# drnatebrown/col-bwt

Measured on AMD Instinct MI355X. Metric: query bases/s, higher is better.
Workload: dtype int64

## Files before the change

### col-bwt_amd/csrc/fat2_query.hip

```cpp
#include <hip/hip_runtime.h>
#include <stdint.h>
#include <stdlib.h>
#include <string.h>

#include <algorithm>

#include "device_layout.h"
#include "fat_cursor.h"
#include "fat_layout.h"
#include "lane_io.h"
#include "lane_out.h"
#include "query_kernels.h"

namespace colbwt {

namespace {

constexpr uint32_t kOffMis0 = 0xFFFFFFFCu;
constexpr uint32_t kOffMis1 = 0xFFFFFFFBu;

#ifdef COLBWT_COUNT_TRIPS
#define FAT2_STAT(k) (++stat[k])
#else
#define FAT2_STAT(k) ((void)0)
#endif

__device__ __forceinline__ uint32_t mis_slot(const uint8_t *top, uint32_t own, uint32_t c) {
    const uint32_t aidx = top[own], cidx = top[c];
    const uint32_t slot = cidx < aidx ? cidx : cidx - 1;
    return cidx < 4 && slot < kFatSlots ? slot : kFatSlots;
}

template <int K, typename PmlT, bool kDeep>
__global__ __launch_bounds__(kQueryBlock)
void fat2_query_kernel(FatTable T, const uint8_t *__restrict__ bases, const uint64_t *__restrict__ read_off,
                       uint64_t n_reads, uint32_t big_reads, uint32_t tail_permille,
                       PmlT *__restrict__ pml, uint8_t *__restrict__ cid) {
    constexpr bool kWide = sizeof(PmlT) == 4;
    __shared__ uint4 s_stage[kWaves][8][64];
    __shared__ uint4 s_win[kWaves][4][64];
    __shared__ uint32_t s_claim;
    __shared__ uint8_t s_top[256];
    const uint32_t wave = threadIdx.x >> 6, lane = threadIdx.x & 63u, g8 = lane & ~7u, p = lane & 7u;
    uint32_t *const s_jx = reinterpret_cast<uint32_t *>(&s_stage[wave][7][48]);
    ChunkPlan plan;
    plan.init(n_reads, big_reads, tail_permille);
    if (threadIdx.x == 0) s_claim = 0;
    s_top[threadIdx.x] = (uint8_t)fat_top_index(T.top4, threadIdx.x);
    __syncthreads();
    uint32_t *const claim = &s_claim;
    ReadCursor rc;
    bool done;
    rc.c_next = threadIdx.x;
    rc.request_chunk(plan, read_off);
    rc.commit();
    done = !rc.enter_chunk(plan, claim);

    OutRuns acc;
    uint32_t trip = 0;
    LaneWindow win;
    win.init(rc.off + rc.k - 1);
    uint4 (*const my_win)[64] = s_win[wave];

    uint32_t j = done ? 0u : T.r - 1;
    uint32_t o = kOffLastPos;
    uint32_t L = 0;
    const uint4 *const my_row = &s_stage[wave][p][g8];

#ifdef COLBWT_COUNT_TRIPS
    unsigned long long stat[8] = {0, 0, 0, 0, 0, 0, 0, 0};
#endif
    while (__any(!done)) {
        bool step_back = false;
        if (!done && rc.k == 0 && !rc.next_in_flight && (rc.r != rc.r_lo || rc.nc_ready)) {
            if (rc.r != rc.r_lo) {
                rc.r -= 1;
                rc.k = rc.off - rc.next_off;
                rc.off = rc.next_off;
                step_back = rc.r > rc.r_lo;
            } else if (kWide || acc.cnt == 0) {
                done = !rc.enter_chunk(plan, claim);
                if (!done) win.init(rc.off + rc.k - 1);
            }
            j = done ? 0u : T.r - 1;
            o = kOffLastPos;
            L = 0;
        }
        const bool live = !done && rc.k != 0;
        uint64_t &k = rc.k;
        const uint64_t g = rc.off + k - 1;

        s_jx[lane] = j;
        wave_sync();
        {
            const uint4 ja = *reinterpret_cast<const uint4 *>(&s_jx[g8]);
            const uint4 jb = *reinterpret_cast<const uint4 *>(&s_jx[g8 + 4]);
            const uint32_t jq[8] = {ja.x, ja.y, ja.z, ja.w, jb.x, jb.y, jb.z, jb.w};
            wave_sync();
#pragma unroll
            for (uint32_t q = 0; q < 8; ++q)
                __builtin_amdgcn_global_load_lds(T.lines + (uint64_t)jq[q] * kFatRowBytes + ((p ^ q) << 4), &s_stage[wave][q][0],
                                                 16, 0, 0);
        }
        if (live && win.avail(g) < (k < 8u ? (uint32_t)k : 8u)) win.request(my_win, bases, g);
        if (step_back) { rc.in_next = read_off[rc.r - 1]; rc.next_in_flight = true; }
        if (!done && rc.fetch_pending) rc.request_chunk(plan, read_off);
        lds_dma_landed();
        rc.commit();

        const uint32_t have = live ? win.avail(g) : 0u;
        uint32_t consumed = 0, l_new = 0, keep = 0xFFFFFFFFu, keep1 = 0xFFFFFFFFu;
        uint64_t ids = 0;
        if (!live || have == 0) FAT2_STAT(5);
        if (live && have != 0) {
            const uint64_t W = win.get8(my_win, lane, g);
            const uint32_t left = k < have ? (uint32_t)k : have;
            if (o == kOffMis0 || o == kOffMis1) {
                FAT2_STAT(2);
                const uint32_t h4 = !kDeep && o == kOffMis1 ? 4u : 0u;
                const uint4 e0 = my_row[(h4 + 0u) ^ p], e1 = my_row[(h4 + 1u) ^ p], e2 = my_row[(h4 + 2u) ^ p],
                            e3 = my_row[(h4 + 3u) ^ p];
                const uint32_t carry = L;
                const uint32_t t1 = (e0.y >> 16) & 0xFFu, d1 = e0.y >> 24, v1 = e3.z & 7u;
                uint32_t oc = 4;
                if (left >= 2) {
                    const uint32_t c2 = (uint32_t)(W >> 48) & 0xFFu;
                    const uint32_t s2 = mis_slot(s_top, t1, c2);
                    if (c2 == t1) oc = 0;
                    else if (s2 < kFatSlots && ((v1 >> s2) & 1u)) oc = 1 + s2;
                }
                if (oc < 4) {
                    const uint32_t J = oc == 0 ? e0.z : oc == 1 ? e0.w : oc == 2 ? e1.x : e1.y;
                    const uint32_t rho = oc == 0 ? e1.z : oc == 1 ? e1.w : oc == 2 ? e2.x : e2.y;
                    const uint32_t pw = oc < 2 ? e2.z : e2.w, P = (oc & 1u) ? pw >> 16 : pw & 0xFFFFu;
                    const uint32_t ch = (e3.x >> (8 * oc)) & 0xFFu, cd = (e3.y >> (8 * oc)) & 0xFFu;
                    const uint32_t vo = (e3.z >> (4 + 4 * oc)) & 7u;
                    consumed = 2;
                    l_new = 1;
                    keep = oc == 0 ? 0xFFFFFFFFu : 0u;
                    ids = (uint64_t)(d1 | (carry << 8));
                    L = oc == 0 ? 1u : 0u;
                    uint32_t nJ = J, nP = P, nrho = rho, nch = ch, ncd = cd, nv = vo, seen = 2;
                    if constexpr (kDeep) {
                        if (left >= 3 && ((uint32_t)(W >> 40) & 0xFFu) == ch) {
                            const uint4 f0 = my_row[4u ^ p], f1 = my_row[5u ^ p], f2 = my_row[6u ^ p], f3 = my_row[7u ^ p];
                            nJ = oc == 0 ? f0.x : oc == 1 ? f0.y : oc == 2 ? f0.z : f0.w;
                            nrho = oc == 0 ? f1.x : oc == 1 ? f1.y : oc == 2 ? f1.z : f1.w;
                            const uint32_t pw2 = oc < 2 ? f2.x : f2.y;
                            nP = (oc & 1u) ? pw2 >> 16 : pw2 & 0xFFFFu;
                            nch = (f2.z >> (8 * oc)) & 0xFFu;
                            ncd = (f2.w >> (8 * oc)) & 0xFFu;
                            nv = (f3.x >> (4 * oc)) & 7u;
                            consumed = 3;
                            seen = 3;
                            ids = (uint64_t)(cd | (d1 << 8) | (carry << 16));
                            if (oc == 0) { l_new = 2; keep = 0xFFFFFFFFu; }
                            else { l_new = 1; keep = 0xFFFFFFFFu; keep1 = 0u; }
                            L += 1;
                        }
                    }
                    if (k > consumed) {
                        uint32_t sn = kFatSlots;
                        if (left > seen) {
                            const uint32_t cn = (uint32_t)(W >> (8u * (7u - seen))) & 0xFFu;
                            if (cn != nch) sn = mis_slot(s_top, nch, cn);
                        }
                        if (sn < kFatSlots && ((nv >> sn) & 1u)) {
                            const uint32_t e = nrho * kFatSlots + sn;
                            j = T.slot_line0 + (kDeep ? e : e >> 1);
                            o = kDeep ? kOffMis0 : kOffMis0 - (e & 1u);
                            L = ncd;
                        } else {
                            j = nJ;
                            o = nP;
                        }
                    }
                } else {
                    consumed = 1;
                    l_new = 0;
                    ids = (uint64_t)carry;
                    L = 0;
                    j = e0.x;
                    o = e0.y & 0xFFFFu;
                }
            } else {
                FAT2_STAT(0);
                const uint4 r0 = my_row[0 ^ p];
                const uint4 r1 = my_row[1 ^ p];
                const uint64_t CH = (uint64_t)r0.x | ((uint64_t)r0.y << 32);
                const uint64_t CID = (uint64_t)r0.z | ((uint64_t)r0.w << 32);
                const uint32_t len = r1.x & 0xFFFFu;
                uint32_t skip = 0;
                bool stay = false;
                if (o == kOffPred) { o = len - 1; skip = 1; }
                else if (o == kOffSucc) { o = 0; skip = 1; }
                else if (o >= len && j < T.r - 1) {
                    o -= len;
                    j += 1;
                    stay = true;
                    FAT2_STAT(1);
                } else {
                    o = o < len ? o : len - 1;
                }
                if (!stay) {
                    const uint64_t X = skip ? ((W >> 8) ^ CH) & 0x00FFFFFFFFFFFFFFull : W ^ CH;
                    const uint32_t run = matching_top_bytes(X);
                    const uint32_t cap = left + skip < (uint32_t)K ? left + skip : (uint32_t)K;
                    uint32_t steps = run < cap ? run : cap;
                    bool own_jump = true, to_entry = false;
                    uint32_t e_next = 0, carry = 0;
                    if (run < cap) {
                        const uint32_t d = run + 1u, sh = 8u * (8u - d);
                        const uint32_t c = (uint32_t)(W >> (sh + 8u * skip)) & 0xFFu;
                        const uint32_t s = mis_slot(s_top, (uint32_t)(CH >> sh) & 0xFFu, c);
                        if (s < kFatSlots && ((r1.w >> (3u * run + s)) & 1u)) {
                            const uint32_t rho = reinterpret_cast<const uint32_t *>(&my_row[((kFatRho / 16) + (run >> 2)) ^ p])[run & 3u];
                            e_next = rho * kFatSlots + s;
                            carry = (uint32_t)(CID >> sh) & 0xFFu;
                            to_entry = true;
                            own_jump = false;
                        }
                    }
                    if (run == 0 && !to_entry) {
                        const uint32_t c = (uint32_t)(W >> 56);
                        const uint32_t cidx = T.cmap[c];
                        bool moved = false;
                        if (cidx != kAbsent) moved = fat_threshold_scan(T, j, o, c, cidx);
                        FAT2_STAT(moved ? 3 : 4);
                        if (moved) {
                            steps = 1;
                            consumed = 1;
                            l_new = 0;
                            own_jump = false;
                        } else {
                            const uint32_t st = matching_top_bytes(X & 0x00FFFFFFFFFFFFFFull);
                            const uint32_t cap0 = left < (uint32_t)K ? left : (uint32_t)K;
                            steps = st < cap0 ? st : cap0;
                            consumed = steps;
                            l_new = steps - 1;
                        }
                    } else {
                        consumed = steps - skip;
                        l_new = L + consumed;
                    }
                    L = l_new;
                    ids = steps ? CID >> (8u * (8u - steps)) : 0ull;
                    if (k == consumed) {
                    } else if (to_entry) {
                        FAT2_STAT(6);
                        j = T.slot_line0 + (kDeep ? e_next : e_next >> 1);
                        o = kDeep ? kOffMis0 : kOffMis0 - (e_next & 1u);
                        L = carry;
                    } else if (own_jump) {
                        const uint32_t e = steps - 1;
                        const uint32_t I = reinterpret_cast<const uint32_t *>(&my_row[((kFatI / 16) + (e >> 2)) ^ p])[e & 3u];
                        const uint32_t Oh = reinterpret_cast<const uint16_t *>(&my_row[((kFatO / 16) + (e >> 3)) ^ p])[e & 7u];
                        const uint64_t cuts = (uint64_t)r1.y | ((uint64_t)r1.z << 32);
                        const uint32_t cut = (uint32_t)(cuts >> (8 * e)) & 0xFFu, cut_a = cut & 0xFu, len_b = cut >> 4;
                        j = I;
                        if (cut_a != kSKCutNone && o >= cut_a) {
                            j += 1;
                            o -= cut_a;
                            if (len_b != kSKCutNone && o >= len_b) {
                                j += 1;
                                o -= len_b;
                            }
                        } else {
                            o += Oh;
                        }
                    }
                }
            }
            if constexpr (kWide) {
                for (uint32_t e = 0; e < consumed; ++e) {
                    pml[g - consumed + 1 + e] = (PmlT)((e < 2 ? keep : keep1) ? l_new - e : 0u);
                    cid[g - consumed + 1 + e] = (uint8_t)(ids >> (8 * e));
                }
            } else {
                acc.push_run(consumed, l_new, keep, keep1, (uint32_t)ids, (uint32_t)(ids >> 32));
            }
            k -= consumed;
        }
        wave_sync();
        if constexpr (!kWide) {
#ifdef COLBWT_ABL_NO_FLUSH
            if ((trip & (OutRuns::kPeriod - 1)) == OutRuns::kPeriod - 1) acc.cnt = acc.cnt > 90 ? 1 : 0;
#else
            if ((trip & (OutRuns::kPeriod - 1)) == OutRuns::kPeriod - 1)
                acc.flush_wave((uint16_t *)pml, cid, rc.off + rc.k, !done, rc.k == 0 && rc.r == rc.r_lo, &s_stage[wave][0][0], lane);
#endif
        }
        ++trip;
        wave_sync();
    }
#ifdef COLBWT_COUNT_TRIPS
    for (int q = 0; q < 8; ++q) atomicAdd(&g_fat_stats[q], stat[q]);
#endif
}

template <int K, typename PmlT, bool kDeep>
uint32_t resident_blocks2() {
    static uint32_t cached[16] = {};
    int dev = 0;
    if (hipGetDevice(&dev) != hipSuccess || dev < 0 || dev >= 16) dev = 0;
    if (cached[dev] == 0) {
        int per_cu = 0, cus = 0;
        if (hipOccupancyMaxActiveBlocksPerMultiprocessor(&per_cu, fat2_query_kernel<K, PmlT, kDeep>, kQueryBlock, 0) != hipSuccess || per_cu < 1)
            per_cu = 1;
        if (hipDeviceGetAttribute(&cus, hipDeviceAttributeMultiprocessorCount, dev) != hipSuccess || cus < 1) cus = 1;
        (void)hipGetLastError();
        cached[dev] = (uint32_t)per_cu * (uint32_t)cus;
    }
    return cached[dev];
}

template <int K, typename PmlT, bool kDeep>
void launch_typed2(const FatTable &T, const uint8_t *d_bases, const uint64_t *d_read_off, uint64_t n_reads, uint64_t n_bases,
                   PmlT *d_pml, uint8_t *d_cid, hipStream_t stream) {
    const uint64_t want_blocks = (n_reads + kQueryBlock - 1) / kQueryBlock;
    const uint32_t blocks = (uint32_t)std::min<uint64_t>(want_blocks, resident_blocks2<K, PmlT, kDeep>());
    const uint64_t lanes = (uint64_t)blocks * kQueryBlock;
    const uint64_t avg_len = std::max<uint64_t>(n_bases / std::max<uint64_t>(n_reads, 1), 1);
    uint32_t big = (uint32_t)std::min<uint64_t>(std::max<uint64_t>(n_bases / lanes / 6 / avg_len, 1), 8);
    uint32_t tail_permille = 100;
    if (const char *e = getenv("COLBWT_LINE_ROWS_CHUNK")) {
        const int v = atoi(e);
        if (v >= 1 && v <= 1024) big = (uint32_t)v;
        if (const char *c = strchr(e, ',')) tail_permille = (uint32_t)std::min(1000, std::max(0, atoi(c + 1)));
    }
    hipLaunchKernelGGL((fat2_query_kernel<K, PmlT, kDeep>), dim3(blocks), dim3(kQueryBlock), 0, stream, T, d_bases, d_read_off, n_reads,
                       big, tail_permille, d_pml, d_cid);
}

template <int K>
void launch_steps2(const FatTable &T, const uint8_t *d_bases, const uint64_t *d_read_off, uint64_t n_reads, uint64_t n_bases,
                   void *d_pml, int pml_bytes, uint8_t *d_cid, hipStream_t stream) {
    const bool deep = T.entry_shift == 7;
    if (pml_bytes == 2 && deep) launch_typed2<K, uint16_t, true>(T, d_bases, d_read_off, n_reads, n_bases, (uint16_t *)d_pml, d_cid, stream);
    else if (pml_bytes == 2) launch_typed2<K, uint16_t, false>(T, d_bases, d_read_off, n_reads, n_bases, (uint16_t *)d_pml, d_cid, stream);
    else if (deep) launch_typed2<K, uint32_t, true>(T, d_bases, d_read_off, n_reads, n_bases, (uint32_t *)d_pml, d_cid, stream);
    else launch_typed2<K, uint32_t, false>(T, d_bases, d_read_off, n_reads, n_bases, (uint32_t *)d_pml, d_cid, stream);
}

}

void launch_fat2_query(const FatTable &T, const uint8_t *d_bases, const uint64_t *d_read_off, uint64_t n_reads, uint64_t n_bases,
                       void *d_pml, int pml_bytes, uint8_t *d_cid, hipStream_t stream) {
    if (n_reads == 0) return;
#define X(K) \
    if (T.steps == K) launch_steps2<K>(T, d_bases, d_read_off, n_reads, n_bases, d_pml, pml_bytes, d_cid, stream);
    COLBWT_FAT_STEPS(X)
#undef X
}

#ifdef COLBWT_COUNT_TRIPS
extern "C" int colbwt_debug_fat2_stats(unsigned long long *out8, int reset) {
    if (hipMemcpyFromSymbol(out8, HIP_SYMBOL(g_fat_stats), 8 * sizeof(unsigned long long)) != hipSuccess) return -1;
    if (reset) {
        unsigned long long z[8] = {0, 0, 0, 0, 0, 0, 0, 0};
        if (hipMemcpyToSymbol(HIP_SYMBOL(g_fat_stats), z, sizeof(z)) != hipSuccess) return -1;
    }
    return 0;
}
#endif

}
```

### col-bwt_amd/csrc/lane_out.h

```cpp
#pragma once
#include <hip/hip_runtime.h>
#include <stdint.h>

#include "lane_io.h"

#ifdef COLBWT_ABL_NO_STORES
#define COLBWT_ABL_IF if (ltop == 0xFFFFFFF1u)
#else
#define COLBWT_ABL_IF
#endif

namespace colbwt {

struct OutRuns {
    static constexpr uint32_t kBlock = 64;
    static constexpr uint32_t kPeriod = 4;
    static constexpr uint32_t kSlotQ = 6, kItemQ = 4;
    static constexpr uint32_t lds_q(uint32_t slots) { return slots * kSlotQ + 2 * slots * kItemQ; }

    uint32_t z0a = 0, z0b = 0, z0c = 0, z1a = 0, z1b = 0, z1c = 0;
    uint32_t ltop = 0;
    uint32_t c0 = 0, c1 = 0, c2 = 0, c3 = 0, c4 = 0, c5 = 0, c6 = 0, c7 = 0, c8 = 0, c9 = 0, c10 = 0, c11 = 0, c12 = 0, c13 = 0, c14 = 0, c15 = 0, c16 = 0, c17 = 0, c18 = 0, c19 = 0, c20 = 0, c21 = 0, c22 = 0, c23 = 0;
    uint32_t cnt = 0;

    __device__ __forceinline__ void push_run(uint32_t n, uint32_t l_new, uint32_t keep, uint32_t keep1, uint32_t ids_lo,
                                             uint32_t ids_hi) {
        const uint32_t in_run = (1u << n) - 1u;
        uint32_t p0 = l_new < n ? 1u << l_new : 0u;
        p0 |= (keep ? 0u : 3u) & in_run;
        p0 |= (keep1 ? 0u : 0xCu) & in_run;
        const uint32_t top = (1u << n) >> 1;
        const uint32_t p1 = (keep & keep1) != 0u && l_new == n ? top : 0u;
        z0c = (uint32_t)(((((uint64_t)z0c << 32) | z0b) << n) >> 32);
        z0b = (uint32_t)(((((uint64_t)z0b << 32) | z0a) << n) >> 32);
        z0a = (z0a << n) | p0;
        z1c = (uint32_t)(((((uint64_t)z1c << 32) | z1b) << n) >> 32);
        z1b = (uint32_t)(((((uint64_t)z1b << 32) | z1a) << n) >> 32);
        z1a = (z1a << n) | p1;
        const bool d4 = n & 8u, d2 = n & 4u;
        c23 = d4 ? c21 : c23;
        c22 = d4 ? c20 : c22;
        c21 = d4 ? c19 : c21;
        c20 = d4 ? c18 : c20;
        c19 = d4 ? c17 : c19;
        c18 = d4 ? c16 : c18;
        c17 = d4 ? c15 : c17;
        c16 = d4 ? c14 : c16;
        c15 = d4 ? c13 : c15;
        c14 = d4 ? c12 : c14;
        c13 = d4 ? c11 : c13;
        c12 = d4 ? c10 : c12;
        c11 = d4 ? c9 : c11;
        c10 = d4 ? c8 : c10;
        c9 = d4 ? c7 : c9;
        c8 = d4 ? c6 : c8;
        c7 = d4 ? c5 : c7;
        c6 = d4 ? c4 : c6;
        c5 = d4 ? c3 : c5;
        c4 = d4 ? c2 : c4;
        c3 = d4 ? c1 : c3;
        c2 = d4 ? c0 : c2;
        c1 = d4 ? 0u : c1;
        c0 = d4 ? 0u : c0;
        c23 = d2 ? c22 : c23;
        c22 = d2 ? c21 : c22;
        c21 = d2 ? c20 : c21;
        c20 = d2 ? c19 : c20;
        c19 = d2 ? c18 : c19;
        c18 = d2 ? c17 : c18;
        c17 = d2 ? c16 : c17;
        c16 = d2 ? c15 : c16;
        c15 = d2 ? c14 : c15;
        c14 = d2 ? c13 : c14;
        c13 = d2 ? c12 : c13;
        c12 = d2 ? c11 : c12;
        c11 = d2 ? c10 : c11;
        c10 = d2 ? c9 : c10;
        c9 = d2 ? c8 : c9;
        c8 = d2 ? c7 : c8;
        c7 = d2 ? c6 : c7;
        c6 = d2 ? c5 : c6;
        c5 = d2 ? c4 : c5;
        c4 = d2 ? c3 : c4;
        c3 = d2 ? c2 : c3;
        c2 = d2 ? c1 : c2;
        c1 = d2 ? c0 : c1;
        c0 = d2 ? 0u : c0;
        const uint32_t sel8 = 0x07060504u - 0x01010101u * (n & 3u);
        c23 = __builtin_amdgcn_perm(c23, c22, sel8);
        c22 = __builtin_amdgcn_perm(c22, c21, sel8);
        c21 = __builtin_amdgcn_perm(c21, c20, sel8);
        c20 = __builtin_amdgcn_perm(c20, c19, sel8);
        c19 = __builtin_amdgcn_perm(c19, c18, sel8);
        c18 = __builtin_amdgcn_perm(c18, c17, sel8);
        c17 = __builtin_amdgcn_perm(c17, c16, sel8);
        c16 = __builtin_amdgcn_perm(c16, c15, sel8);
        c15 = __builtin_amdgcn_perm(c15, c14, sel8);
        c14 = __builtin_amdgcn_perm(c14, c13, sel8);
        c13 = __builtin_amdgcn_perm(c13, c12, sel8);
        c12 = __builtin_amdgcn_perm(c12, c11, sel8);
        c11 = __builtin_amdgcn_perm(c11, c10, sel8);
        c10 = __builtin_amdgcn_perm(c10, c9, sel8);
        c9 = __builtin_amdgcn_perm(c9, c8, sel8);
        c8 = __builtin_amdgcn_perm(c8, c7, sel8);
        c7 = __builtin_amdgcn_perm(c7, c6, sel8);
        c6 = __builtin_amdgcn_perm(c6, c5, sel8);
        c5 = __builtin_amdgcn_perm(c5, c4, sel8);
        c4 = __builtin_amdgcn_perm(c4, c3, sel8);
        c3 = __builtin_amdgcn_perm(c3, c2, sel8);
        c2 = __builtin_amdgcn_perm(c2, c1, sel8);
        c1 = __builtin_amdgcn_perm(c1, c0, sel8);
        c0 = __builtin_amdgcn_perm(c0, 0u, sel8);
        const uint32_t mlo = n >= 4 ? 0xFFFFFFFFu : (1u << (8 * n)) - 1u;
        const uint32_t mhi = n >= 8 ? 0xFFFFFFFFu : (n > 4 ? (1u << (8 * (n - 4))) - 1u : 0u);
        c0 |= ids_lo & mlo;
        c1 |= ids_hi & mhi;
        cnt += n;
    }

    static __device__ __forceinline__ void shr96(uint64_t &lo, uint32_t &hi, uint32_t s) {
        if (s >= 64) {
            lo = (uint64_t)(hi >> (s - 64));
            hi = 0;
        } else if (s) {
            lo = (lo >> s) | ((uint64_t)hi << (64 - s));
            hi = s < 32 ? hi >> s : 0u;
        }
    }
    static __device__ __forceinline__ uint64_t low64_from(uint32_t a, uint32_t b, uint32_t c, uint32_t s) {
        uint64_t lo = ((uint64_t)b << 32) | a;
        uint32_t hi = c;
        shr96(lo, hi, s);
        return lo;
    }
    __device__ __forceinline__ uint32_t park_item(uint4 *item, uint32_t slot, uint32_t e_lo, uint32_t count, uint64_t addr, uint32_t lt) const {
        const uint32_t o_lo = (uint32_t)addr & (kBlock - 1), o_hi = o_lo + count;
        const uint64_t in_item = count >= 64 ? ~0ull : (1ull << count) - 1ull;
        const uint64_t Z0 = (low64_from(z0a, z0b, z0c, e_lo) & in_item) << o_lo;
        const uint64_t Z1 = (low64_from(z1a, z1b, z1c, e_lo) & in_item) << o_lo;
        const uint32_t z0w[2] = {(uint32_t)Z0, (uint32_t)(Z0 >> 32)}, z1w[2] = {(uint32_t)Z1, (uint32_t)(Z1 >> 32)};
        uint32_t pm[8];
        uint32_t v = lt;
#pragma unroll
        for (int p = 7; p >= 0; --p) {
            const uint32_t b0 = (z0w[p >> 2] >> (8 * (p & 3))) & 0xFFu, b1 = (z1w[p >> 2] >> (8 * (p & 3))) & 0xFFu;
            pm[p] = (v & 0xFFFFu) | (b0 << 16) | (b1 << 24);
            const uint32_t lo_p = o_lo > 8u * p ? o_lo : 8u * p, hi_p = o_hi < 8u * p + 8u ? o_hi : 8u * p + 8u;
            if (hi_p > lo_p) {
                const uint32_t bits = b0 | b1;
                if (bits) {
                    const uint32_t q = (uint32_t)__builtin_ctz(bits);
                    v = q - (lo_p - 8u * p) + ((b1 >> q) & 1u);
                } else {
                    v += hi_p - lo_p;
                }
            }
        }
        item[0] = make_uint4(slot, e_lo, count, (uint32_t)addr);
        item[1] = make_uint4((uint32_t)(addr >> 32), 0u, 0u, 0u);
        item[2] = make_uint4(pm[0], pm[1], pm[2], pm[3]);
        item[3] = make_uint4(pm[4], pm[5], pm[6], pm[7]);
        return v;
    }

    template <uint32_t kSlots = 32>
    __device__ __forceinline__ void flush_wave(uint16_t *pml, uint8_t *cid, uint64_t gl, bool active, bool final, uint4 *lds,
                                               uint32_t lane) {
        constexpr uint32_t kItemBase = kSlots * kSlotQ;
        const uint32_t below = (0u - (uint32_t)gl) & (kBlock - 1);
        const bool has_a = active && below < cnt;
        const uint32_t rest = below < cnt ? below : cnt;
        const bool has_b = active && final && rest != 0;
        const unsigned long long emit = __ballot(has_a || has_b);
        if (emit == 0) return;
        const uint32_t n_a = has_a ? cnt - below : 0u;
        uint32_t v_cut = ltop;
        const unsigned long long lt = (1ull << lane) - 1ull;
        const uint32_t rank = (uint32_t)__builtin_popcountll(emit & lt), lanes = (uint32_t)__builtin_popcountll(emit);
        for (uint32_t first = 0; first < lanes; first += kSlots) {
            const bool mine = (has_a || has_b) && rank >= first && rank < first + kSlots;
            const bool rag_a = mine && has_a && n_a != kBlock, rag_b = mine && has_b, full_a = mine && has_a && n_a == kBlock;
            const unsigned long long m_ra = __ballot(rag_a), m_rb = __ballot(rag_b), m_fa = __ballot(full_a);
            const uint32_t n_ra = (uint32_t)__builtin_popcountll(m_ra), n_rb = (uint32_t)__builtin_popcountll(m_rb);
            const uint32_t n_rag = n_ra + n_rb, n_items = n_rag + (uint32_t)__builtin_popcountll(m_fa);
            if (mine) {
                uint4 *slot = lds + kSlotQ * (rank - first);
                slot[0] = make_uint4(c0, c1, c2, c3);
                slot[1] = make_uint4(c4, c5, c6, c7);
                slot[2] = make_uint4(c8, c9, c10, c11);
                slot[3] = make_uint4(c12, c13, c14, c15);
                slot[4] = make_uint4(c16, c17, c18, c19);
                slot[5] = make_uint4(c20, c21, c22, c23);
            }
#pragma unroll 1
            for (uint32_t which = 0; which < 2; ++which) {
                const bool b_item = which != 0;
                if (!__any(mine && (b_item ? has_b : has_a))) continue;
                if (mine && (b_item ? has_b : has_a)) {
                    const uint32_t at = b_item ? n_ra + (uint32_t)__builtin_popcountll(m_rb & lt)
                                               : (rag_a ? (uint32_t)__builtin_popcountll(m_ra & lt) : n_rag + (uint32_t)__builtin_popcountll(m_fa & lt));
                    const uint32_t v_low = park_item(lds + kItemBase + kItemQ * at, rank - first, b_item ? 0u : below, b_item ? rest : n_a,
                                                     b_item ? gl : gl + below, b_item ? v_cut : ltop);
                    if (!b_item) v_cut = v_low;
                }
            }
            wave_sync();
            for (uint32_t t = lane; t < 8u * n_items; t += 64) {
                const uint32_t it = t >> 3, piece = t & 7u;
                const uint4 *item = lds + kItemBase + kItemQ * it;
                const uint4 h = item[0];
                const uint64_t addr = (uint64_t)h.w | ((uint64_t)item[1].x << 32), end = addr + h.z;
                const uint64_t w0 = (addr & ~(uint64_t)(kBlock - 1)) + 8u * piece;
                if (w0 < addr || w0 + 8u > end) continue;
                const uint32_t d = reinterpret_cast<const uint32_t *>(item + 2)[piece];
                const uint32_t b0 = (d >> 16) & 0xFFu, b1 = d >> 24;
                uint32_t v = d & 0xFFFFu;
                uint32_t out[4] = {0, 0, 0, 0};
#pragma unroll
                for (int i = 7; i >= 0; --i) {
                    v = (b1 >> i) & 1u ? 1u : ((b0 >> i) & 1u ? 0u : v + 1u);
                    out[i >> 1] |= (v & 0xFFFFu) << (16 * (i & 1));
                }
                COLBWT_ABL_IF *reinterpret_cast<uint4 *>(pml + w0) = make_uint4(out[0], out[1], out[2], out[3]);
            }
            for (uint32_t t = lane; t < 4u * n_items; t += 64) {
                const uint32_t it = t >> 2, piece = t & 3u;
                const uint4 *item = lds + kItemBase + kItemQ * it;
                const uint4 h = item[0];
                const uint64_t addr = (uint64_t)h.w | ((uint64_t)item[1].x << 32), end = addr + h.z;
                const uint64_t w0 = (addr & ~(uint64_t)(kBlock - 1)) + 16u * piece;
                if (w0 < addr || w0 + 16u > end) continue;
                const uint32_t e = h.y + (uint32_t)(w0 - addr);
                const uint32_t *bytes = reinterpret_cast<const uint32_t *>(lds + kSlotQ * h.x);
                const uint32_t dq = e >> 2, sel = 0x03020100u + 0x01010101u * (e & 3u);
                const uint32_t x0 = bytes[dq], x1 = bytes[dq + 1], x2 = bytes[dq + 2], x3 = bytes[dq + 3], x4 = bytes[dq + 4 < 24u ? dq + 4 : 23u];
                COLBWT_ABL_IF *reinterpret_cast<uint4 *>(cid + w0) =
                    make_uint4(__builtin_amdgcn_perm(x1, x0, sel), __builtin_amdgcn_perm(x2, x1, sel), __builtin_amdgcn_perm(x3, x2, sel),
                               __builtin_amdgcn_perm(x4, x3, sel));
            }
            for (uint32_t t = lane; t < 16u * n_rag; t += 64) {
                const uint32_t it = t >> 4, i = t & 7u;
                const bool tail = (t >> 3) & 1u;
                const uint4 *item = lds + kItemBase + kItemQ * it;
                const uint4 h = item[0];
                const uint64_t addr = (uint64_t)h.w | ((uint64_t)item[1].x << 32), end = addr + h.z;
                const uint64_t w_head = addr & ~7ull, w_tail = end & ~7ull;
                if (tail ? ((end & 7u) == 0 || (w_tail == w_head && (addr & 7u) != 0)) : (addr & 7u) == 0) continue;
                const uint64_t w0 = tail ? w_tail : w_head, el = w0 + i;
                if (el < addr || el >= end) continue;
                const uint32_t piece = (uint32_t)(w0 >> 3) & 7u;
                const uint32_t d = reinterpret_cast<const uint32_t *>(item + 2)[piece];
                const uint32_t b0 = (d >> 16) & 0xFFu, b1 = d >> 24, bits = (b0 | b1) >> i;
                const uint32_t hi = end - w0 < 8u ? (uint32_t)(end - w0) : 8u;
                uint32_t v;
                if (bits) {
                    const uint32_t q = (uint32_t)__builtin_ctz(bits);
                    v = q + ((b1 >> (i + q)) & 1u);
                } else {
                    v = (d & 0xFFFFu) + hi - i;
                }
                COLBWT_ABL_IF pml[el] = (uint16_t)v;
            }
            for (uint32_t t = lane; t < 32u * n_rag; t += 64) {
                const uint32_t it = t >> 5, i = t & 15u;
                const bool tail = (t >> 4) & 1u;
                const uint4 *item = lds + kItemBase + kItemQ * it;
                const uint4 h = item[0];
                const uint64_t addr = (uint64_t)h.w | ((uint64_t)item[1].x << 32), end = addr + h.z;
                const uint64_t w_head = addr & ~15ull, w_tail = end & ~15ull;
                if (tail ? ((end & 15u) == 0 || (w_tail == w_head && (addr & 15u) != 0)) : (addr & 15u) == 0) continue;
                const uint64_t el = (tail ? w_tail : w_head) + i;
                if (el < addr || el >= end) continue;
                COLBWT_ABL_IF cid[el] = reinterpret_cast<const uint8_t *>(lds + kSlotQ * h.x)[h.y + (uint32_t)(el - addr)];
            }
            wave_sync();
        }
        if (has_a || has_b) {
            if (final) {
                z0a = z0b = z0c = z1a = z1b = z1c = 0;
                ltop = 0;
                cnt = 0;
            } else {
                ltop = v_cut;
                const uint64_t keep_lo = (1ull << below) - 1ull;
                z0a &= (uint32_t)keep_lo; z0b &= (uint32_t)(keep_lo >> 32); z0c = 0;
                z1a &= (uint32_t)keep_lo; z1b &= (uint32_t)(keep_lo >> 32); z1c = 0;
                cnt = below;
            }
        }
    }
};

}
```

Before: 142.0 billion.

## Replace per-step register shift accumulator with per-trip records assembled at flush

Each trip now stores its output as a small record (ids plus a packed mask word) in one of four register slots, instead of shifting 24 id registers and 96-bit masks on every step. At flush time each lane assembles its byte image and masks in its own LDS slot, then reloads the carried bytes from that slot. The shared flush logic moves into a common OutFlush helper, and the staging LDS grows to hold per-lane images. This removes the per-trip perm and shift chain, at the cost of more LDS, a switch on the trip index, and extra LDS traffic during flush.

After: 143.4 billion, median of 6. Within noise of the previous version (+1.0%).

```diff
diff --git a/col-bwt_amd/csrc/fat2_query.hip b/col-bwt_amd/csrc/fat2_query.hip
--- a/col-bwt_amd/csrc/fat2_query.hip
+++ b/col-bwt_amd/csrc/fat2_query.hip
@@ -16,6 +16,8 @@
 
 namespace {
 
+static_assert(OutRecs::kLdsQ % 64 == 0 && OutRecs::kLdsQ >= 8 * 64, "the flush's working area holds the staged lines");
+
 constexpr uint32_t kOffMis0 = 0xFFFFFFFCu;
 constexpr uint32_t kOffMis1 = 0xFFFFFFFBu;
 
@@ -37,7 +39,7 @@
                        uint64_t n_reads, uint32_t big_reads, uint32_t tail_permille,
                        PmlT *__restrict__ pml, uint8_t *__restrict__ cid) {
     constexpr bool kWide = sizeof(PmlT) == 4;
-    __shared__ uint4 s_stage[kWaves][8][64];
+    __shared__ uint4 s_stage[kWaves][OutRecs::kLdsQ / 64][64];
     __shared__ uint4 s_win[kWaves][4][64];
     __shared__ uint32_t s_claim;
     __shared__ uint8_t s_top[256];
@@ -56,7 +58,7 @@
     rc.commit();
     done = !rc.enter_chunk(plan, claim);
 
-    OutRuns acc;
+    OutRecs acc;
     uint32_t trip = 0;
     LaneWindow win;
     win.init(rc.off + rc.k - 1);
@@ -276,17 +278,16 @@
                     pml[g - consumed + 1 + e] = (PmlT)((e < 2 ? keep : keep1) ? l_new - e : 0u);
                     cid[g - consumed + 1 + e] = (uint8_t)(ids >> (8 * e));
                 }
-            } else {
-                acc.push_run(consumed, l_new, keep, keep1, (uint32_t)ids, (uint32_t)(ids >> 32));
             }
             k -= consumed;
         }
+        if constexpr (!kWide) acc.push(trip & (OutRecs::kPeriod - 1), consumed, l_new, keep, keep1, (uint32_t)ids, (uint32_t)(ids >> 32));
         wave_sync();
         if constexpr (!kWide) {
 #ifdef COLBWT_ABL_NO_FLUSH
-            if ((trip & (OutRuns::kPeriod - 1)) == OutRuns::kPeriod - 1) acc.cnt = acc.cnt > 90 ? 1 : 0;
+            if ((trip & (OutRecs::kPeriod - 1)) == OutRecs::kPeriod - 1) acc.cnt = acc.cnt > 90 ? 1 : 0;
 #else
-            if ((trip & (OutRuns::kPeriod - 1)) == OutRuns::kPeriod - 1)
+            if ((trip & (OutRecs::kPeriod - 1)) == OutRecs::kPeriod - 1)
                 acc.flush_wave((uint16_t *)pml, cid, rc.off + rc.k, !done, rc.k == 0 && rc.r == rc.r_lo, &s_stage[wave][0][0], lane);
 #endif
         }
diff --git a/col-bwt_amd/csrc/lane_out.h b/col-bwt_amd/csrc/lane_out.h
--- a/col-bwt_amd/csrc/lane_out.h
+++ b/col-bwt_amd/csrc/lane_out.h
@@ -12,10 +12,171 @@
 
 namespace colbwt {
 
+struct OutFlush {
+    static constexpr uint32_t kBlock = 64;
+    static constexpr uint32_t kSlotQ = 6, kItemQ = 4;
+
+    struct Masks {
+        uint32_t z0a, z0b, z0c, z1a, z1b, z1c;
+    };
+
+    static __device__ __forceinline__ void shr96(uint64_t &lo, uint32_t &hi, uint32_t s) {
+        if (s >= 64) {
+            lo = (uint64_t)(hi >> (s - 64));
+            hi = 0;
+        } else if (s) {
+            lo = (lo >> s) | ((uint64_t)hi << (64 - s));
+            hi = s < 32 ? hi >> s : 0u;
+        }
+    }
+    static __device__ __forceinline__ uint64_t low64_from(uint32_t a, uint32_t b, uint32_t c, uint32_t s) {
+        uint64_t lo = ((uint64_t)b << 32) | a;
+        uint32_t hi = c;
+        shr96(lo, hi, s);
+        return lo;
+    }
+    static __device__ __forceinline__ uint32_t park_item(uint4 *item, const Masks &m, uint32_t slot, uint32_t e_lo, uint32_t byte0,
+                                                         uint32_t count, uint64_t addr, uint32_t lt) {
+        const uint32_t o_lo = (uint32_t)addr & (kBlock - 1), o_hi = o_lo + count;
+        const uint64_t in_item = count >= 64 ? ~0ull : (1ull << count) - 1ull;
+        const uint64_t Z0 = (low64_from(m.z0a, m.z0b, m.z0c, e_lo) & in_item) << o_lo;
+        const uint64_t Z1 = (low64_from(m.z1a, m.z1b, m.z1c, e_lo) & in_item) << o_lo;
+        const uint32_t z0w[2] = {(uint32_t)Z0, (uint32_t)(Z0 >> 32)}, z1w[2] = {(uint32_t)Z1, (uint32_t)(Z1 >> 32)};
+        uint32_t pm[8];
+        uint32_t v = lt;
+#pragma unroll
+        for (int p = 7; p >= 0; --p) {
+            const uint32_t b0 = (z0w[p >> 2] >> (8 * (p & 3))) & 0xFFu, b1 = (z1w[p >> 2] >> (8 * (p & 3))) & 0xFFu;
+            pm[p] = (v & 0xFFFFu) | (b0 << 16) | (b1 << 24);
+            const uint32_t lo_p = o_lo > 8u * p ? o_lo : 8u * p, hi_p = o_hi < 8u * p + 8u ? o_hi : 8u * p + 8u;
+            if (hi_p > lo_p) {
+                const uint32_t bits = b0 | b1;
+                if (bits) {
+                    const uint32_t q = (uint32_t)__builtin_ctz(bits);
+                    v = q - (lo_p - 8u * p) + ((b1 >> q) & 1u);
+                } else {
+                    v += hi_p - lo_p;
+                }
+            }
+        }
+        item[0] = make_uint4(slot, byte0 + e_lo, count, (uint32_t)addr);
+        item[1] = make_uint4((uint32_t)(addr >> 32), 0u, 0u, 0u);
+        item[2] = make_uint4(pm[0], pm[1], pm[2], pm[3]);
+        item[3] = make_uint4(pm[4], pm[5], pm[6], pm[7]);
+        return v;
+    }
+
+    template <uint32_t kSlots, bool kLaneImages, class Dump>
+    static __device__ __forceinline__ uint32_t emit(uint16_t *pml, uint8_t *cid, uint64_t gl, bool has_a, bool has_b, uint32_t below,
+                                                    uint32_t cnt, uint32_t ltop, const Masks &m, uint32_t byte0, uint4 *lds,
+                                                    uint32_t lane, Dump dump) {
+        constexpr uint32_t kItemBase = (kLaneImages ? 64u : kSlots) * kSlotQ;
+        const unsigned long long emit = __ballot(has_a || has_b);
+        uint32_t v_cut = ltop;
+        if (emit == 0) return v_cut;
+        const uint32_t n_a = has_a ? cnt - below : 0u;
+        const uint32_t rest = below < cnt ? below : cnt;
+        const unsigned long long lt = (1ull << lane) - 1ull;
+        const uint32_t rank = (uint32_t)__builtin_popcountll(emit & lt), lanes = (uint32_t)__builtin_popcountll(emit);
+        for (uint32_t first = 0; first < lanes; first += kSlots) {
+            const bool mine = (has_a || has_b) && rank >= first && rank < first + kSlots;
+            const uint32_t slot = kLaneImages ? lane : rank - first;
+            const bool rag_a = mine && has_a && n_a != kBlock, rag_b = mine && has_b, full_a = mine && has_a && n_a == kBlock;
+            const unsigned long long m_ra = __ballot(rag_a), m_rb = __ballot(rag_b), m_fa = __ballot(full_a);
+            const uint32_t n_ra = (uint32_t)__builtin_popcountll(m_ra), n_rb = (uint32_t)__builtin_popcountll(m_rb);
+            const uint32_t n_rag = n_ra + n_rb, n_items = n_rag + (uint32_t)__builtin_popcountll(m_fa);
+            if (!kLaneImages && mine) dump(lds + kSlotQ * slot);
+#pragma unroll 1
+            for (uint32_t which = 0; which < 2; ++which) {
+                const bool b_item = which != 0;
+                if (!__any(mine && (b_item ? has_b : has_a))) continue;
+                if (mine && (b_item ? has_b : has_a)) {
+                    const uint32_t at = b_item ? n_ra + (uint32_t)__builtin_popcountll(m_rb & lt)
+                                               : (rag_a ? (uint32_t)__builtin_popcountll(m_ra & lt) : n_rag + (uint32_t)__builtin_popcountll(m_fa & lt));
+                    const uint32_t v_low = park_item(lds + kItemBase + kItemQ * at, m, slot, b_item ? 0u : below, byte0, b_item ? rest : n_a,
+                                                     b_item ? gl : gl + below, b_item ? v_cut : ltop);
+                    if (!b_item) v_cut = v_low;
+                }
+            }
+            wave_sync();
+            for (uint32_t t = lane; t < 8u * n_items; t += 64) {
+                const uint32_t it = t >> 3, piece = t & 7u;
+                const uint4 *item = lds + kItemBase + kItemQ * it;
+                const uint4 h = item[0];
+                const uint64_t addr = (uint64_t)h.w | ((uint64_t)item[1].x << 32), end = addr + h.z;
+                const uint64_t w0 = (addr & ~(uint64_t)(kBlock - 1)) + 8u * piece;
+                if (w0 < addr || w0 + 8u > end) continue;
+                const uint32_t d = reinterpret_cast<const uint32_t *>(item + 2)[piece];
+                const uint32_t b0 = (d >> 16) & 0xFFu, b1 = d >> 24;
+                uint32_t v = d & 0xFFFFu;
+                uint32_t out[4] = {0, 0, 0, 0};
+#pragma unroll
+                for (int i = 7; i >= 0; --i) {
+                    v = (b1 >> i) & 1u ? 1u : ((b0 >> i) & 1u ? 0u : v + 1u);
+                    out[i >> 1] |= (v & 0xFFFFu) << (16 * (i & 1));
+                }
+                COLBWT_ABL_IF *reinterpret_cast<uint4 *>(pml + w0) = make_uint4(out[0], out[1], out[2], out[3]);
+            }
+            for (uint32_t t = lane; t < 4u * n_items; t += 64) {
+                const uint32_t it = t >> 2, piece = t & 3u;
+                const uint4 *item = lds + kItemBase + kItemQ * it;
+                const uint4 h = item[0];
+                const uint64_t addr = (uint64_t)h.w | ((uint64_t)item[1].x << 32), end = addr + h.z;
+                const uint64_t w0 = (addr & ~(uint64_t)(kBlock - 1)) + 16u * piece;
+                if (w0 < addr || w0 + 16u > end) continue;
+                const uint32_t e = h.y + (uint32_t)(w0 - addr);
+                const uint32_t *bytes = reinterpret_cast<const uint32_t *>(lds + kSlotQ * h.x);
+                const uint32_t dq = e >> 2, sel = 0x03020100u + 0x01010101u * (e & 3u);
+                const uint32_t x0 = bytes[dq], x1 = bytes[dq + 1], x2 = bytes[dq + 2], x3 = bytes[dq + 3], x4 = bytes[dq + 4 < 24u ? dq + 4 : 23u];
+                COLBWT_ABL_IF *reinterpret_cast<uint4 *>(cid + w0) =
+                    make_uint4(__builtin_amdgcn_perm(x1, x0, sel), __builtin_amdgcn_perm(x2, x1, sel), __builtin_amdgcn_perm(x3, x2, sel),
+                               __builtin_amdgcn_perm(x4, x3, sel));
+            }
+            for (uint32_t t = lane; t < 16u * n_rag; t += 64) {
+                const uint32_t it = t >> 4, i = t & 7u;
+                const bool tail = (t >> 3) & 1u;
+                const uint4 *item = lds + kItemBase + kItemQ * it;
+                const uint4 h = item[0];
+                const uint64_t addr = (uint64_t)h.w | ((uint64_t)item[1].x << 32), end = addr + h.z;
+                const uint64_t w_head = addr & ~7ull, w_tail = end & ~7ull;
+                if (tail ? ((end & 7u) == 0 || (w_tail == w_head && (addr & 7u) != 0)) : (addr & 7u) == 0) continue;
+                const uint64_t w0 = tail ? w_tail : w_head, el = w0 + i;
+                if (el < addr || el >= end) continue;
+                const uint32_t piece = (uint32_t)(w0 >> 3) & 7u;
+                const uint32_t d = reinterpret_cast<const uint32_t *>(item + 2)[piece];
+                const uint32_t b0 = (d >> 16) & 0xFFu, b1 = d >> 24, bits = (b0 | b1) >> i;
+                const uint32_t hi = end - w0 < 8u ? (uint32_t)(end - w0) : 8u;
+                uint32_t v;
+                if (bits) {
+                    const uint32_t q = (uint32_t)__builtin_ctz(bits);
+                    v = q + ((b1 >> (i + q)) & 1u);
+                } else {
+                    v = (d & 0xFFFFu) + hi - i;
+                }
+                COLBWT_ABL_IF pml[el] = (uint16_t)v;
+            }
+            for (uint32_t t = lane; t < 32u * n_rag; t += 64) {
+                const uint32_t it = t >> 5, i = t & 15u;
+                const bool tail = (t >> 4) & 1u;
+                const uint4 *item = lds + kItemBase + kItemQ * it;
+                const uint4 h = item[0];
+                const uint64_t addr = (uint64_t)h.w | ((uint64_t)item[1].x << 32), end = addr + h.z;
+                const uint64_t w_head = addr & ~15ull, w_tail = end & ~15ull;
+                if (tail ? ((end & 15u) == 0 || (w_tail == w_head && (addr & 15u) != 0)) : (addr & 15u) == 0) continue;
+                const uint64_t el = (tail ? w_tail : w_head) + i;
+                if (el < addr || el >= end) continue;
+                COLBWT_ABL_IF cid[el] = reinterpret_cast<const uint8_t *>(lds + kSlotQ * h.x)[h.y + (uint32_t)(el - addr)];
+            }
+            wave_sync();
+        }
+        return v_cut;
+    }
+};
+
 struct OutRuns {
-    static constexpr uint32_t kBlock = 64;
+    static constexpr uint32_t kBlock = OutFlush::kBlock;
     static constexpr uint32_t kPeriod = 4;
-    static constexpr uint32_t kSlotQ = 6, kItemQ = 4;
+    static constexpr uint32_t kSlotQ = OutFlush::kSlotQ, kItemQ = OutFlush::kItemQ;
     static constexpr uint32_t lds_q(uint32_t slots) { return slots * kSlotQ + 2 * slots * kItemQ; }
 
     uint32_t z0a = 0, z0b = 0, z0c = 0, z1a = 0, z1b = 0, z1c = 0;
@@ -118,163 +279,22 @@
         cnt += n;
     }
 
-    static __device__ __forceinline__ void shr96(uint64_t &lo, uint32_t &hi, uint32_t s) {
-        if (s >= 64) {
-            lo = (uint64_t)(hi >> (s - 64));
-            hi = 0;
-        } else if (s) {
-            lo = (lo >> s) | ((uint64_t)hi << (64 - s));
-            hi = s < 32 ? hi >> s : 0u;
-        }
-    }
-    static __device__ __forceinline__ uint64_t low64_from(uint32_t a, uint32_t b, uint32_t c, uint32_t s) {
-        uint64_t lo = ((uint64_t)b << 32) | a;
-        uint32_t hi = c;
-        shr96(lo, hi, s);
-        return lo;
-    }
-    __device__ __forceinline__ uint32_t park_item(uint4 *item, uint32_t slot, uint32_t e_lo, uint32_t count, uint64_t addr, uint32_t lt) const {
-        const uint32_t o_lo = (uint32_t)addr & (kBlock - 1), o_hi = o_lo + count;
-        const uint64_t in_item = count >= 64 ? ~0ull : (1ull << count) - 1ull;
-        const uint64_t Z0 = (low64_from(z0a, z0b, z0c, e_lo) & in_item) << o_lo;
-        const uint64_t Z1 = (low64_from(z1a, z1b, z1c, e_lo) & in_item) << o_lo;
-        const uint32_t z0w[2] = {(uint32_t)Z0, (uint32_t)(Z0 >> 32)}, z1w[2] = {(uint32_t)Z1, (uint32_t)(Z1 >> 32)};
-        uint32_t pm[8];
-        uint32_t v = lt;
-#pragma unroll
-        for (int p = 7; p >= 0; --p) {
-            const uint32_t b0 = (z0w[p >> 2] >> (8 * (p & 3))) & 0xFFu, b1 = (z1w[p >> 2] >> (8 * (p & 3))) & 0xFFu;
-            pm[p] = (v & 0xFFFFu) | (b0 << 16) | (b1 << 24);
-            const uint32_t lo_p = o_lo > 8u * p ? o_lo : 8u * p, hi_p = o_hi < 8u * p + 8u ? o_hi : 8u * p + 8u;
-            if (hi_p > lo_p) {
-                const uint32_t bits = b0 | b1;
-                if (bits) {
-                    const uint32_t q = (uint32_t)__builtin_ctz(bits);
-                    v = q - (lo_p - 8u * p) + ((b1 >> q) & 1u);
-                } else {
-                    v += hi_p - lo_p;
-                }
-            }
-        }
-        item[0] = make_uint4(slot, e_lo, count, (uint32_t)addr);
-        item[1] = make_uint4((uint32_t)(addr >> 32), 0u, 0u, 0u);
-        item[2] = make_uint4(pm[0], pm[1], pm[2], pm[3]);
-        item[3] = make_uint4(pm[4], pm[5], pm[6], pm[7]);
-        return v;
-    }
-
     template <uint32_t kSlots = 32>
     __device__ __forceinline__ void flush_wave(uint16_t *pml, uint8_t *cid, uint64_t gl, bool active, bool final, uint4 *lds,
                                                uint32_t lane) {
-        constexpr uint32_t kItemBase = kSlots * kSlotQ;
         const uint32_t below = (0u - (uint32_t)gl) & (kBlock - 1);
         const bool has_a = active && below < cnt;
         const uint32_t rest = below < cnt ? below : cnt;
         const bool has_b = active && final && rest != 0;
-        const unsigned long long emit = __ballot(has_a || has_b);
-        if (emit == 0) return;
-        const uint32_t n_a = has_a ? cnt - below : 0u;
-        uint32_t v_cut = ltop;
-        const unsigned long long lt = (1ull << lane) - 1ull;
-        const uint32_t rank = (uint32_t)__builtin_popcountll(emit & lt), lanes = (uint32_t)__builtin_popcountll(emit);
-        for (uint32_t first = 0; first < lanes; first += kSlots) {
-            const bool mine = (has_a || has_b) && rank >= first && rank < first + kSlots;
-            const bool rag_a = mine && has_a && n_a != kBlock, rag_b = mine && has_b, full_a = mine && has_a && n_a == kBlock;
-            const unsigned long long m_ra = __ballot(rag_a), m_rb = __ballot(rag_b), m_fa = __ballot(full_a);
-            const uint32_t n_ra = (uint32_t)__builtin_popcountll(m_ra), n_rb = (uint32_t)__builtin_popcountll(m_rb);
-            const uint32_t n_rag = n_ra + n_rb, n_items = n_rag + (uint32_t)__builtin_popcountll(m_fa);
-            if (mine) {
-                uint4 *slot = lds + kSlotQ * (rank - first);
-                slot[0] = make_uint4(c0, c1, c2, c3);
-                slot[1] = make_uint4(c4, c5, c6, c7);
-                slot[2] = make_uint4(c8, c9, c10, c11);
-                slot[3] = make_uint4(c12, c13, c14, c15);
-                slot[4] = make_uint4(c16, c17, c18, c19);
-                slot[5] = make_uint4(c20, c21, c22, c23);
-            }
-#pragma unroll 1
-            for (uint32_t which = 0; which < 2; ++which) {
-                const bool b_item = which != 0;
-                if (!__any(mine && (b_item ? has_b : has_a))) continue;
-                if (mine && (b_item ? has_b : has_a)) {
-                    const uint32_t at = b_item ? n_ra + (uint32_t)__builtin_popcountll(m_rb & lt)
-                                               : (rag_a ? (uint32_t)__builtin_popcountll(m_ra & lt) : n_rag + (uint32_t)__builtin_popcountll(m_fa & lt));
-                    const uint32_t v_low = park_item(lds + kItemBase + kItemQ * at, rank - first, b_item ? 0u : below, b_item ? rest : n_a,
-                                                     b_item ? gl : gl + below, b_item ? v_cut : ltop);
-                    if (!b_item) v_cut = v_low;
-                }
-            }
-            wave_sync();
-            for (uint32_t t = lane; t < 8u * n_items; t += 64) {
-                const uint32_t it = t >> 3, piece = t & 7u;
-                const uint4 *item = lds + kItemBase + kItemQ * it;
-                const uint4 h = item[0];
-                const uint64_t addr = (uint64_t)h.w | ((uint64_t)item[1].x << 32), end = addr + h.z;
-                const uint64_t w0 = (addr & ~(uint64_t)(kBlock - 1)) + 8u * piece;
-                if (w0 < addr || w0 + 8u > end) continue;
-                const uint32_t d = reinterpret_cast<const uint32_t *>(item + 2)[piece];
-                const uint32_t b0 = (d >> 16) & 0xFFu, b1 = d >> 24;
-                uint32_t v = d & 0xFFFFu;
-                uint32_t out[4] = {0, 0, 0, 0};
-#pragma unroll
-                for (int i = 7; i >= 0; --i) {
-                    v = (b1 >> i) & 1u ? 1u : ((b0 >> i) & 1u ? 0u : v + 1u);
-                    out[i >> 1] |= (v & 0xFFFFu) << (16 * (i & 1));
-                }
-                COLBWT_ABL_IF *reinterpret_cast<uint4 *>(pml + w0) = make_uint4(out[0], out[1], out[2], out[3]);
-            }
-            for (uint32_t t = lane; t < 4u * n_items; t += 64) {
-                const uint32_t it = t >> 2, piece = t & 3u;
-                const uint4 *item = lds + kItemBase + kItemQ * it;
-                const uint4 h = item[0];
-                const uint64_t addr = (uint64_t)h.w | ((uint64_t)item[1].x << 32), end = addr + h.z;
-                const uint64_t w0 = (addr & ~(uint64_t)(kBlock - 1)) + 16u * piece;
-                if (w0 < addr || w0 + 16u > end) continue;
-                const uint32_t e = h.y + (uint32_t)(w0 - addr);
-                const uint32_t *bytes = reinterpret_cast<const uint32_t *>(lds + kSlotQ * h.x);
-                const uint32_t dq = e >> 2, sel = 0x03020100u + 0x01010101u * (e & 3u);
-                const uint32_t x0 = bytes[dq], x1 = bytes[dq + 1], x2 = bytes[dq + 2], x3 = bytes[dq + 3], x4 = bytes[dq + 4 < 24u ? dq + 4 : 23u];
-                COLBWT_ABL_IF *reinterpret_cast<uint4 *>(cid + w0) =
-                    make_uint4(__builtin_amdgcn_perm(x1, x0, sel), __builtin_amdgcn_perm(x2, x1, sel), __builtin_amdgcn_perm(x3, x2, sel),
-                               __builtin_amdgcn_perm(x4, x3, sel));
-            }
-            for (uint32_t t = lane; t < 16u * n_rag; t += 64) {
-                const uint32_t it = t >> 4, i = t & 7u;
-                const bool tail = (t >> 3) & 1u;
-                const uint4 *item = lds + kItemBase + kItemQ * it;
-                const uint4 h = item[0];
-                const uint64_t addr = (uint64_t)h.w | ((uint64_t)item[1].x << 32), end = addr + h.z;
-                const uint64_t w_head = addr & ~7ull, w_tail = end & ~7ull;
-                if (tail ? ((end & 7u) == 0 || (w_tail == w_head && (addr & 7u) != 0)) : (addr & 7u) == 0) continue;
-                const uint64_t w0 = tail ? w_tail : w_head, el = w0 + i;
-                if (el < addr || el >= end) continue;
-                const uint32_t piece = (uint32_t)(w0 >> 3) & 7u;
-                const uint32_t d = reinterpret_cast<const uint32_t *>(item + 2)[piece];
-                const uint32_t b0 = (d >> 16) & 0xFFu, b1 = d >> 24, bits = (b0 | b1) >> i;
-                const uint32_t hi = end - w0 < 8u ? (uint32_t)(end - w0) : 8u;
-                uint32_t v;
-                if (bits) {
-                    const uint32_t q = (uint32_t)__builtin_ctz(bits);
-                    v = q + ((b1 >> (i + q)) & 1u);
-                } else {
-                    v = (d & 0xFFFFu) + hi - i;
-                }
-                COLBWT_ABL_IF pml[el] = (uint16_t)v;
-            }
-            for (uint32_t t = lane; t < 32u * n_rag; t += 64) {
-                const uint32_t it = t >> 5, i = t & 15u;
-                const bool tail = (t >> 4) & 1u;
-                const uint4 *item = lds + kItemBase + kItemQ * it;
-                const uint4 h = item[0];
-                const uint64_t addr = (uint64_t)h.w | ((uint64_t)item[1].x << 32), end = addr + h.z;
-                const uint64_t w_head = addr & ~15ull, w_tail = end & ~15ull;
-                if (tail ? ((end & 15u) == 0 || (w_tail == w_head && (addr & 15u) != 0)) : (addr & 15u) == 0) continue;
-                const uint64_t el = (tail ? w_tail : w_head) + i;
-                if (el < addr || el >= end) continue;
-                COLBWT_ABL_IF cid[el] = reinterpret_cast<const uint8_t *>(lds + kSlotQ * h.x)[h.y + (uint32_t)(el - addr)];
-            }
-            wave_sync();
-        }
+        const OutFlush::Masks m = {z0a, z0b, z0c, z1a, z1b, z1c};
+        const uint32_t v_cut = OutFlush::emit<kSlots, false>(pml, cid, gl, has_a, has_b, below, cnt, ltop, m, 0u, lds, lane, [&](uint4 *slot) {
+            slot[0] = make_uint4(c0, c1, c2, c3);
+            slot[1] = make_uint4(c4, c5, c6, c7);
+            slot[2] = make_uint4(c8, c9, c10, c11);
+            slot[3] = make_uint4(c12, c13, c14, c15);
+            slot[4] = make_uint4(c16, c17, c18, c19);
+            slot[5] = make_uint4(c20, c21, c22, c23);
+        });
         if (has_a || has_b) {
             if (final) {
                 z0a = z0b = z0c = z1a = z1b = z1c = 0;
@@ -291,4 +311,97 @@
     }
 };
 
+struct OutRecs {
+    static constexpr uint32_t kBlock = OutFlush::kBlock;
+    static constexpr uint32_t kPeriod = 4;
+    static constexpr uint32_t kSlots = 24;
+    static constexpr uint32_t kCarryByte = 32;
+    static constexpr uint32_t kLdsQ = 64 * OutFlush::kSlotQ + 2 * kSlots * OutFlush::kItemQ;
+
+    uint32_t r0l = 0, r0h = 0, r0d = 0, r1l = 0, r1h = 0, r1d = 0, r2l = 0, r2h = 0, r2d = 0, r3l = 0, r3h = 0, r3d = 0;
+    uint32_t k0 = 0, k1 = 0, k2 = 0, k3 = 0, k4 = 0, k5 = 0, k6 = 0, k7 = 0, k8 = 0, k9 = 0, k10 = 0, k11 = 0, k12 = 0, k13 = 0, k14 = 0, k15 = 0;
+    uint64_t y0 = 0, y1 = 0;
+    uint32_t ltop = 0;
+    uint32_t cnt = 0;
+
+    __device__ __forceinline__ void push(uint32_t t, uint32_t n, uint32_t l_new, uint32_t keep, uint32_t keep1, uint32_t ids_lo,
+                                         uint32_t ids_hi) {
+        const uint32_t in_run = (1u << n) - 1u;
+        uint32_t p0 = l_new < n ? 1u << l_new : 0u;
+        p0 |= (keep ? 0u : 3u) & in_run;
+        p0 |= (keep1 ? 0u : 0xCu) & in_run;
+        const uint32_t top = (1u << n) >> 1;
+        const uint32_t p1 = (keep & keep1) != 0u && l_new == n ? top : 0u;
+        const uint32_t d = n | (p0 << 8) | (p1 << 16);
+        cnt += n;
+        switch (t) {
+        case 0: r0l = ids_lo; r0h = ids_hi; r0d = d; break;
+        case 1: r1l = ids_lo; r1h = ids_hi; r1d = d; break;
+        case 2: r2l = ids_lo; r2h = ids_hi; r2d = d; break;
+        default: r3l = ids_lo; r3h = ids_hi; r3d = d; break;
+        }
+    }
+
+    static __device__ __forceinline__ void put8(uint8_t *at, uint32_t lo, uint32_t hi) {
+        const uint64_t v = (uint64_t)lo | ((uint64_t)hi << 32);
+        __builtin_memcpy(at, &v, 8);
+    }
+
+    __device__ __forceinline__ void flush_wave(uint16_t *pml, uint8_t *cid, uint64_t gl, bool active, bool final, uint4 *lds,
+                                               uint32_t lane) {
+        const uint32_t n0 = r0d & 0xFFu, n1 = r1d & 0xFFu, n2 = r2d & 0xFFu, n3 = r3d & 0xFFu;
+        const uint32_t e2 = n3, e1 = e2 + n2, e0 = e1 + n1, N = e0 + n0;
+        const uint32_t s = kCarryByte - N;
+        uint4 *const slot = lds + OutFlush::kSlotQ * lane;
+        uint8_t *const img = reinterpret_cast<uint8_t *>(slot);
+        put8(img + s, r3l, r3h);
+        put8(img + s + e2, r2l, r2h);
+        put8(img + s + e1, r1l, r1h);
+        put8(img + s + e0, r0l, r0h);
+        slot[2] = make_uint4(k0, k1, k2, k3);
+        slot[3] = make_uint4(k4, k5, k6, k7);
+        slot[4] = make_uint4(k8, k9, k10, k11);
+        slot[5] = make_uint4(k12, k13, k14, k15);
+        const uint32_t q0 = ((r3d >> 8) & 0xFFu) | (((r2d >> 8) & 0xFFu) << e2) | (((r1d >> 8) & 0xFFu) << e1) | (((r0d >> 8) & 0xFFu) << e0);
+        const uint32_t q1 = (r3d >> 16) | ((r2d >> 16) << e2) | ((r1d >> 16) << e1) | ((r0d >> 16) << e0);
+        const uint64_t Z0 = (y0 << N) | q0, Z1 = (y1 << N) | q1;
+        const OutFlush::Masks m = {(uint32_t)Z0, (uint32_t)(Z0 >> 32), (uint32_t)((y0 >> 1) >> (63 - N)),
+                                   (uint32_t)Z1, (uint32_t)(Z1 >> 32), (uint32_t)((y1 >> 1) >> (63 - N))};
+        const uint32_t below = (0u - (uint32_t)gl) & (kBlock - 1);
+        const bool has_a = active && below < cnt;
+        const uint32_t rest = below < cnt ? below : cnt;
+        const bool has_b = active && final && rest != 0;
+        const uint32_t v_cut = OutFlush::emit<kSlots, true>(pml, cid, gl, has_a, has_b, below, cnt, ltop, m, s, lds, lane, [](uint4 *) {});
+        const bool sent = has_a || has_b;
+        const uint32_t kept = sent ? (final ? 0u : below) : cnt;
+        if (sent) ltop = final ? 0u : v_cut;
+        cnt = kept;
+        const uint64_t keep_lo = (1ull << kept) - 1ull;
+        y0 = (((uint64_t)m.z0b << 32) | m.z0a) & keep_lo;
+        y1 = (((uint64_t)m.z1b << 32) | m.z1a) & keep_lo;
+        const uint32_t *w = reinterpret_cast<const uint32_t *>(img);
+        const uint32_t dq = s >> 2, sel = 0x03020100u + 0x01010101u * (s & 3u);
+        uint32_t x[17];
+#pragma unroll
+        for (uint32_t i = 0; i < 16; ++i) x[i] = w[dq + i];
+        x[16] = w[dq + 16 < 24u ? dq + 16 : 23u];
+        k0 = __builtin_amdgcn_perm(x[1], x[0], sel);
+        k1 = __builtin_amdgcn_perm(x[2], x[1], sel);
+        k2 = __builtin_amdgcn_perm(x[3], x[2], sel);
+        k3 = __builtin_amdgcn_perm(x[4], x[3], sel);
+        k4 = __builtin_amdgcn_perm(x[5], x[4], sel);
+        k5 = __builtin_amdgcn_perm(x[6], x[5], sel);
+        k6 = __builtin_amdgcn_perm(x[7], x[6], sel);
+        k7 = __builtin_amdgcn_perm(x[8], x[7], sel);
+        k8 = __builtin_amdgcn_perm(x[9], x[8], sel);
+        k9 = __builtin_amdgcn_perm(x[10], x[9], sel);
+        k10 = __builtin_amdgcn_perm(x[11], x[10], sel);
+        k11 = __builtin_amdgcn_perm(x[12], x[11], sel);
+        k12 = __builtin_amdgcn_perm(x[13], x[12], sel);
+        k13 = __builtin_amdgcn_perm(x[14], x[13], sel);
+        k14 = __builtin_amdgcn_perm(x[15], x[14], sel);
+        k15 = __builtin_amdgcn_perm(x[16], x[15], sel);
+    }
+};
+
 }
```
